# wenxichen/tensorflow_yolo2

Hardware: AMD Instinct MI355X
Metric: images/sec fwd+bwd Darknet-19 416x416 (higher is better)
Workload: dtype f16; 1 GPU; YOLO detector train step: darknet19_core + darknet19_detection(30) + get_loss + backward + Adam; image_size=416, batch_per_gpu=64, global_batch=64, S=13, B=2, parallelism=dp1, grad_allreduce=none

## Files before the change

### tensorflow_yolo2_amd/csrc/conv_halo.hip

```cpp
#include <stdio.h>
#include <stdlib.h>

#include <algorithm>

#include "common.h"
#include "conv_epilogue.h"
#include "kernels.h"

namespace y2 {

template <typename T, int WP, int WC, int TP, int TC, int BKB, int NSB, bool ADB>
struct HaloCfg {
    static constexpr int NW = WP * WC, NT = NW * 64;
    static constexpr int BP = WP * TP * 32, BC = WC * TC * 32;
    static constexpr int SZ = sizeof(T);
    static constexpr int LPR = BKB / 16, RPI = 64 / LPR, RPB = 256 / BKB;
    static constexpr int NI_C = BC / RPI;
    static constexpr int IPWB = (NI_C + NW - 1) / NW;
    static constexpr int IPW_MIN = NI_C / NW;
    static constexpr int BSTAGE = BC * BKB;
    static constexpr int KG = BKB / 32;
    static constexpr int NA = ADB ? 2 : 1;
};

// ... 403 lines not shown
    if (dtype == 3 && !no_pl2 && kb == 64) k128 = true;
    const int bkb = k128 ? 128 : 64;
    if (a.Cout > 64) {
        constexpr long kCUs = 256;
        const long wgs = (long)((a.M + 127) / 128) * ((a.Cout + 127) / 128);
        return conv_tile(2, 4, 2, 1, bkb, !dtype_split(dtype) && k128 && wgs <= kCUs ? 3 : 2);
    }
    return a.Cout > 32 ? conv_tile(4, 1, 2, 2, bkb, 2) : conv_tile(4, 1, 2, 1, bkb, 2);
}

#ifdef Y2_DEVBUILD
static int dev_rule(int W, int Cout) {
    static int n = -1;
    static int rules[32][3];
    if (n < 0) {
        n = 0;
        const char* e = getenv("Y2DEV_CONV");
        while (e && *e && n < 32) {
            int w, c, v, used = 0;
            if (sscanf(e, "%d:%d:%d%n", &w, &c, &v, &used) != 3) break;
            rules[n][0] = w; rules[n][1] = c; rules[n][2] = v; ++n;
            e += used;
            if (*e == ',') ++e;
        }
    }
    for (int i = 0; i < n; ++i)
        if (rules[i][0] == W && rules[i][1] == Cout) return rules[i][2];
    return -1;
}
#endif

static ConvPlan plan_route(int dtype, const ConvArgs& a) {
    ConvPlan p{CK_IGEMM, 0, 0, 0, 1};
    const int kb = a.C * dtype_kbytes(dtype);
    const bool split = dtype_split(dtype);
    const int rf = rf_config(a.taps, a.W, kb, a.Cout, a.M);
    const int rfn = rfn_config(a.taps, a.W, kb, a.Cout, a.M, a.is_dgrad, a.bw_psum != nullptr);
    if ((dtype == 1 || dtype == 2) && ((!a.bw_psum && rf) || rfn)) {
        p.kind = rf && !a.bw_psum ? CK_RF : CK_RFN;
        p.cfg = p.kind == CK_RF ? rf : rfn;
        const RfForm f = rf_form(p.cfg, a.bw_psum != nullptr);
        const int ntiles = (int)(((long)a.N * (a.H + 1) * (a.W + 1) + f.bp - 1) / f.bp);
        const int nblk = std::min((f.lds <= 80 * 1024 ? 512 : 256) / ((a.Cout + f.bc - 1) / f.bc), ntiles);
        p.rf_tiles = (ntiles + nblk - 1) / nblk;
        p.records = (ntiles + p.rf_tiles - 1) / p.rf_tiles;
        p.block_pixels = f.bp;
        p.lds = f.lds;
        return p;
    }
    if (a.taps == 9 && !(!split && (rf || rfn)) && (a.W <= 104 || a.Cout <= 32)) {
        p.kind = CK_HALOQ;
        p.cfg = haloq_tile(dtype, a, kb);
        p.filter_layout = ConvTile(p.cfg).aux ? 2 : 1;
        p.block_pixels = ConvTile(p.cfg).bp();
        if (p.cfg == HQ_256x64 && !split && a.M < 384 * 8) {
            const int depth = ks_clamp(ks_depth(((a.M + 255) / 256) * ((a.Cout + 63) / 64), 128, kb / 128), a);
            if (depth >= 2 && (size_t)image_rows(ConvTile(p.cfg), a, 0) * 128 <= (size_t)kLdsMax) {
                p.kind = CK_HALOQ_KS;
                p.ks_depth = depth;
                p.block_pixels = 128;
            }
        }
        return p;
    }
#ifdef Y2_DEVBUILD
    if (a.taps == 9 && dtype == 1 && dev_rule(a.W, a.Cout) >= 0) {
// ... 7 lines not shown
        p.kind = CK_HALO;
        p.cfg = halo_tile(dtype, a, kb);
        p.block_pixels = ConvTile(p.cfg).bp();
        return p;
    }
    p.cfg = igemm_tile(dtype, a, kb);
    p.block_pixels = ConvTile(p.cfg).bp();
    if (a.taps == 1 && dtype <= 2 && a.M < 384 * 8 && kb % 128 == 0 && a.Cout > 64) {
        const int depth = ks_clamp(ks_depth(((a.M + 127) / 128) * ((a.Cout + 127) / 128), 48, kb / 128), a);
        if (depth >= 2) {
            p.kind = CK_IGEMM_KS;
            p.cfg = conv_tile(2, 4, 2, 1, 128, 2);
            p.ks_depth = depth;
        }
    }
    return p;
}
ConvPlan plan_conv(int dtype, const ConvArgs& a) {
    ConvPlan p = plan_route(dtype, a);
    if (p.kind != CK_RF && p.kind != CK_RFN) p.records = (a.M + p.block_pixels - 1) / p.block_pixels;
    return p;
}

hipError_t launch_conv(int dtype, const ConvArgs& a0, hipStream_t s, int filter_layout) {
    static const int xcd_mode = getenv("Y2_XCD_CONV") ? atoi(getenv("Y2_XCD_CONV")) : 1;
    ConvArgs a = a0;
    a.xcd = xcd_mode;
    const ConvPlan p = plan_conv(dtype, a);
    if (filter_layout != p.filter_layout) return hipErrorInvalidValue;
    switch (p.kind) {
        case CK_RF: case CK_RFN: return launch_conv_rf(dtype, p, a, s);
        case CK_HALOQ: case CK_HALOQ_KS: return launch_conv_haloq(dtype, p, a, s);
        case CK_HALO: return launch_conv_halo(dtype, p, a, s);
        default: return launch_conv_igemm(dtype, p, a, s);
    }
}

#ifdef Y2_DEVBUILD
#define HV(id, WP, TPARGS...) \
    case id: if (bp) *bp = halo_bp<WP, TPARGS>(); return run ? halo_pick<T, WP, TPARGS>(a, s) : hipSuccess;
template <int WP, int WC, int TP, int TC, int BKB, int NSB, int ABL = 0>
static constexpr int halo_bp() { return WP * TP * 32; }
hipError_t launch_conv_halo_variant(int variant, const ConvArgs& a, hipStream_t s, int* bp, bool run) {
    typedef half_t T;
    switch (variant) {
        HV(86, 4, 2, 4, 1, 64, 2)
        HV(87, 4, 2, 3, 1, 64, 2)
        HV(88, 4, 2, 2, 1, 64, 2)
        HV(89, 4, 1, 4, 1, 128, 2)
        HV(90, 8, 1, 2, 1, 128, 2)
        HV(91, 8, 1, 4, 1, 128, 2)
        HV(92, 8, 1, 2, 1, 64, 2)
        HV(93, 8, 1, 4, 1, 64, 2)
        HV(94, 4, 2, 4, 2, 128, 2)
        HV(95, 8, 1, 2, 2, 128, 2)
        HV(96, 8, 1, 2, 2, 64, 2)
        HV(20, 2, 2, 2, 2, 128, 3)
        HV(21, 2, 2, 2, 2, 128, 2)
        HV(22, 2, 4, 2, 1, 128, 3)
        HV(23, 2, 4, 2, 1, 128, 2)
        HV(24, 4, 2, 2, 2, 128, 3)
        HV(25, 2, 4, 2, 2, 128, 3)
        HV(26, 2, 4, 2, 2, 128, 2)
        HV(27, 2, 2, 2, 2, 128, 4)
        HV(28, 2, 2, 2, 2, 64, 3)
        HV(29, 2, 2, 2, 2, 64, 2)
// ... 52 lines not shown
```

### tensorflow_yolo2_amd/csrc/kernels.h

```cpp
#pragma once
#include <hip/hip_runtime.h>
#include <stddef.h>
#include <stdint.h>
#include "../../include/yolo2_hip.h"

namespace y2 {

inline size_t dtype_size(int dtype) { return (dtype == 0 || dtype >= 3) ? 4 : 2; }
inline int dtype_kbytes(int dtype) { return dtype == 0 ? 4 : 2; }
inline bool dtype_split(int dtype) { return dtype >= 3; }
inline int dtype_plain(int dtype) { return dtype >= 3 ? 0 : dtype; }

struct ConvArgs {
    const void* x;
    const void* w;
    void* y;
    const float* bias;
    float* part_cnt;
    float* part_mean;
    float* part_m2;
    int N, H, W, C;
    int M;
    int Cout;
    int ldy;
    int taps;
    const void* bw_y = nullptr;
    const float* bw_scale = nullptr;
    const float* bw_shift = nullptr;
    float* bw_psum = nullptr;
    float bw_slope = 0.1f;
    unsigned* nonfinite = nullptr;
    int xcd = 0;
    int is_dgrad = 0;
    const float* aff_scale = nullptr;
    const float* aff_shift = nullptr;
    void* aff_out = nullptr;
    float aff_slope = 0.1f;
    uint32_t aff_magW = 0, aff_magH = 0;
    int aff_shW = 0, aff_shH = 0;
    int aff_pool = 0;
    float* ks_scratch = nullptr;
    size_t ks_floats = 0;
    int ks_splits = 0;
};
size_t conv_ks_scratch_floats(int taps, int M, int ldy, int row_bytes);
inline void conv_div_magic(uint32_t d, uint32_t* mag, int* sh) {
    int l = 0;
    while ((1u << l) < d) ++l;
    *sh = 31 + l;
    *mag = (uint32_t)((((uint64_t)1 << (31 + l)) + d - 1) / d);
}
inline void conv_set_affine(ConvArgs& a, const float* scale, const float* shift, void* out_bordered) {
    a.aff_scale = scale; a.aff_shift = shift; a.aff_out = out_bordered;
    conv_div_magic((uint32_t)a.W, &a.aff_magW, &a.aff_shW);
    conv_div_magic((uint32_t)a.H, &a.aff_magH, &a.aff_shH);
}

enum ConvKind {
    CK_RF,
    CK_RFN,
    CK_HALOQ,
    CK_HALOQ_KS,
    CK_HALO,
    CK_IGEMM,
    CK_IGEMM_KS,
};
struct ConvPlan {
    ConvKind kind;
    int cfg;
    int filter_layout;
    int block_pixels;
    int ks_depth;
    int records;
    int rf_tiles;
    int lds;
};
constexpr int rf_lds(int sz, int C, int nct, int wp, int tp, int pr) {
    return 4 * wp * tp * 32 * C * sz + wp * pr * (nct * 32 * sz + 16) + wp * (2 * nct * 32 + 2) * 8 + nct * 32 * 4;
}
constexpr int rfn_lds(int sz, int C, int wp, int wn, int tp, int nslot, bool bw) {
    const int bp = wp * tp * 32, bc = wn * 32, nw = wp * wn;
    return nslot * bp * C * sz + bp * (bc * sz + 16) + 2 * (nw * 2 * bc + nw) * 4 + bp * 4 + bc * 4 +
           (bw ? bp * bc * sz + 2 * bc * 4 : 0);
}
constexpr int conv_tile(int wp, int wc, int tp, int tc, int bkb, int aux) {
    return wp | wc << 4 | tp << 8 | tc << 12 | (bkb / 64) << 16 | aux << 20;
}
struct ConvTile {
    int wp, wc, tp, tc, bkb, aux;
    explicit ConvTile(int t)
        : wp(t & 15), wc((t >> 4) & 15), tp((t >> 8) & 15), tc((t >> 12) & 15), bkb(((t >> 16) & 15) * 64), aux(t >> 20) {}
    int bp() const { return wp * tp * 32; }
    int bc() const { return wc * tc * 32; }
};
ConvPlan plan_conv(int dtype, const ConvArgs& a);
hipError_t launch_conv(int dtype, const ConvArgs& a, hipStream_t s, int filter_layout);
hipError_t launch_conv_rf(int dtype, const ConvPlan& p, const ConvArgs& a, hipStream_t s);
hipError_t launch_conv_haloq(int dtype, const ConvPlan& p, const ConvArgs& a, hipStream_t s);
hipError_t launch_conv_halo(int dtype, const ConvPlan& p, const ConvArgs& a, hipStream_t s);
hipError_t launch_conv_igemm(int dtype, const ConvPlan& p, const ConvArgs& a, hipStream_t s);
int halo_image_rows(int H, int W, int BP, int RPI, int pool = 0);
int conv_block_couts(int Cout);
int mx8_block_couts();
int mx8_channels(int C);
struct Mx8Out {
    uint8_t* q = nullptr;
    uint8_t* sc = nullptr;
    int ldq = 0;
};
hipError_t launch_conv_mx8(int out_f32, const ConvArgs& a, const uint8_t* xsc, const uint8_t* wsc, const Mx8Out* qo,
                           hipStream_t s);
hipError_t launch_mx_unpack(const uint8_t* q, const uint8_t* sc, float* out, int N, int H, int W, int C, int Cs,
                            hipStream_t s);
hipError_t launch_mx_quantize(int in_f16, const void* x, size_t rows, int ldin, int ldq, uint8_t* q, uint8_t* sc,
                              hipStream_t s);
hipError_t launch_mx_pack_filter(const float* w, int taps, int Cin, int Cout, int Cout_pad, int C8, uint8_t* q,
                                 uint8_t* sc, hipStream_t s);

enum Conv1Fwd {
    C1F_PLAIN,
    C1F_POOLED,
};
enum Conv1Stats {
    C1S_NONE,
    C1S_CONV,
    C1S_GRAM,
};
enum Conv1Keep {
    C1K_NONE,
    C1K_Y,
    C1K_YSEL,
    C1K_IDX3,
};
// ... 412 lines not shown
```

### tensorflow_yolo2_amd/csrc/net.hip

```cpp
#include <math.h>
#include <stdarg.h>
#include <stdio.h>
#include <string.h>

#include <algorithm>
#include <string>
#include <vector>

#include "../../include/yolo2_hip.h"
#include "common.h"
#include "kernels.h"
#include "optim_math.h"

using namespace y2;

static thread_local std::string g_err;
namespace y2 {
int set_error(int code, const char* msg) {
    g_err = msg;
    return code;
}
}
static int fail(int code, const char* fmt, ...) {
    char buf[512];
// ... 7 lines not shown
#define HIPCHK(expr)                                                                                  \
    do {                                                                                              \
        hipError_t _e = (expr);                                                                       \
        if (_e != hipSuccess) return fail(Y2_ERR_HIP, "%s: %s (%s:%d)", #expr, hipGetErrorString(_e), \
                                          __FILE__, __LINE__);                                        \
    } while (0)

static inline size_t align_up(size_t v, size_t a) { return (v + a - 1) / a * a; }
static inline int round_up(int v, int a) { return (v + a - 1) / a * a; }

static inline size_t part_rows_bound(int N, int H, int W, int cout) {
    const size_t bp = 64;
    return ((size_t)N * (H + 1) * (W + 1) + bp - 1) / bp;
}

struct PadGeom {
    int N, H, W, C;
    size_t front_px() const { return (size_t)W + 3; }
    size_t body_px() const { return bbody_pixels(N, H, W); }
    size_t back_px() const { return (size_t)2 * W + 6 + 256; }
    size_t bytes(size_t sz) const { return align_up((front_px() + body_px() + back_px()) * C * sz + 64, 256); }
    size_t base_off(size_t sz) const { return front_px() * C * sz; }
};

struct Layer {
    int k, cin, cout, pool;
    int H, W, Ho, Wo, M;
    int cin_s;
    int ldy;
    int cout_pad;
    int cin_pad;
    bool first3;
    int wf_frag = 0, wd_frag = 0;
    float slope = 0.1f;
    size_t pW, pb, pg, pbeta;
    size_t smm, smv;
    size_t xin, y, stat, wf, wd, dyp, ysel, idx0;
    int cin8 = 0;
    size_t x8 = 0, x8s = 0, w8 = 0, w8s = 0;
};

enum FwdFold { FOLD_NONE, FOLD_AFFINE, FOLD_AFFINE_POOL };
enum FwdStats {
    FS_MOVING,
    FS_CONV,
    FS_SUB,
    FS_GRAM,
};
enum FwdApply {
    FA_NONE,
    FA_ACT,
    FA_FIN_ACT,
    FA_CONV1_POOL,
};
enum FwdOut { OUT_NEXT, OUT_EXT, OUT_F32, OUT_H32 };
enum BwdReduce {
    BR_KERNEL,
    BR_DGRAD,
    BR_CONV1_LIN,
    BR_CONV1_RECOMPUTE,
};
enum BwdApply { BA_FIN_APPLY, BA_FIN_THEN_APPLY, BA_FIN };
enum WgradRoute { WG_GENERIC, WG_CONV1, WG_CONV1_FUSED, WG_CONV1_LIN };
struct LayerPlan {
    int training = 0;
    bool mx8 = false;
    bool in8 = false;
    bool out8 = false;
    FwdFold fold = FOLD_NONE;
    FwdStats stats = FS_MOVING;
    int P = 0;
    FwdApply apply = FA_ACT;
    FwdOut out = OUT_NEXT;
    BwdReduce bred = BR_KERNEL;
    int bP = 0;
    BwdApply bapply = BA_FIN_THEN_APPLY;
    WgradRoute wgrad = WG_GENERIC;
    bool wgrad_side = false;
    bool dgrad = false;
    int dgrad_dtype = 0;
    bool dgrad_fuse = false;
    bool dgrad_guard = false;
    ConvPlan dgrad_plan{};
};
struct NetPlan {
    int train_core = 0, train_head = 0;
    std::vector<LayerPlan> L;
    Conv1Plan c1{};
};

struct y2_ctx {
    int N, H, W, dtype, tail, tail_k, core_layers;
    int bwd_dtype = 0;
    int fp8 = 0;
    int mx8_all = 0;
    std::vector<Layer> L;
    size_t nparams = 0, nstate = 0;
    int outN, outH, outW, outC;
    float grad_scale = 1.f;
    int bessel = 0;
    float bn_eps = 1e-3f, bn_momentum = 0.99f;
    int zero_bias_grad = 0;
// ... 53 lines not shown
    std::vector<ProfRec> prof_recs;
    size_t prof_used = 0;
    size_t sz() const { return dtype_size(dtype); }
    PadGeom in_geom(int l) const { return PadGeom{N, L[l].H, L[l].W, L[l].cin_s}; }
    PadGeom dy_geom(int l) const { return PadGeom{N, L[l].H, L[l].W, L[l].ldy}; }
    Conv1Plan conv1_plan(bool trains, bool training) const {
        const Layer& y = L[0];
        return plan_conv1(dtype, bwd_dtype, N, y.H, y.W, y.pool, y.cout, y.ldy, trains, L.size() > 1, training);
    }
};

enum { CAT_CONV_FWD = 0, CAT_CONV1_FWD, CAT_DGRAD, CAT_WGRAD, CAT_CONV1_WGRAD, CAT_BN_FWD, CAT_BN_BWD, CAT_MISC,
       CAT_COUNT };

struct ProfScope {
    y2_ctx* c; hipStream_t s; int idx = -1;
    ProfScope(y2_ctx* c_, hipStream_t s_, int cat) : c(c_), s(s_) {
        if (!c->prof) return;
        if (c->prof == 2 && cat != CAT_CONV_FWD && cat != CAT_DGRAD && cat != CAT_WGRAD) return;
        if (c->prof_used == c->prof_recs.size()) {
            y2_ctx::ProfRec r; r.cat = cat;
            if (hipEventCreate(&r.a) != hipSuccess || hipEventCreate(&r.b) != hipSuccess) return;
            c->prof_recs.push_back(r);
        }
        idx = (int)c->prof_used++;
        c->prof_recs[idx].cat = cat;
        c->prof_recs[idx].layer = c->prof_layer;
        (void)hipEventRecord(c->prof_recs[idx].a, s);
    }
    ~ProfScope() { if (idx >= 0) (void)hipEventRecord(c->prof_recs[idx].b, s); }
};
#define PROF(cat) ProfScope _prof_scope(c, s, cat)

static ConvArgs fwd_args(const y2_ctx* c, int l, bool stats, FwdFold fold) {
    const Layer& y = c->L[l];
    const size_t sz = c->sz();
    ConvArgs a{};
    a.x = (l == 0 && c->ext_xin) ? (char*)c->ext_xin : c->ws + y.xin + c->in_geom(l).base_off(sz);
    a.w = c->ws + y.wf; a.y = c->ws + y.y; a.bias = c->params + y.pb;
    if (stats) {
        a.part_cnt = (float*)(c->ws + c->o_part_cnt); a.part_mean = (float*)(c->ws + c->o_part_mean);
        a.part_m2 = (float*)(c->ws + c->o_part_m2);
    }
    a.N = c->N; a.H = y.H; a.W = y.W; a.C = y.cin_s; a.M = y.M; a.Cout = y.cout; a.ldy = y.ldy;
    a.taps = y.k * y.k;
    if (c->ks_floats) { a.ks_scratch = (float*)(c->ws + c->o_ks); a.ks_floats = c->ks_floats; }
    if (fold != FOLD_NONE) {
        const float* stat = (const float*)(c->ws + y.stat);
        conv_set_affine(a, stat, stat + y.ldy, c->ws + c->L[l + 1].xin + c->in_geom(l + 1).base_off(sz));
        a.aff_slope = y.slope;
        a.aff_pool = fold == FOLD_AFFINE_POOL ? 1 : 0;
    }
    return a;
}
static ConvArgs dgrad_args(const y2_ctx* c, int l, bool fuse, bool guard) {
    const Layer& y = c->L[l];
    ConvArgs a{};
    a.x = c->ws + y.dyp + c->dy_geom(l).base_off(c->sz()); a.w = c->ws + y.wd;
    a.N = c->N; a.H = y.H; a.W = y.W; a.C = y.ldy; a.M = y.M; a.Cout = y.cin; a.ldy = y.cin;
    a.taps = y.k * y.k;
    a.is_dgrad = 1;
    if (c->ks_floats) { a.ks_scratch = (float*)(c->ws + c->o_ks); a.ks_floats = c->ks_floats; }
    if (guard) a.nonfinite = (unsigned*)(c->ws + c->o_nfflag);
    if (fuse) {
        const Layer& z = c->L[l - 1];
        float* zs = (float*)(c->ws + z.stat);
        a.bw_y = c->ws + (z.pool ? z.ysel : z.y);
        a.bw_scale = zs; a.bw_shift = zs + z.ldy; a.bw_psum = (float*)(c->ws + c->o_psum);
        a.bw_slope = z.slope;
    }
    return a;
}
static int dgrad_dtype(const y2_ctx* c, int l) {
    return c->bwd_dtype == 4 && l > 0 && !c->L[l - 1].first3 ? 5 : c->bwd_dtype;
}

static bool mx8_speed_ok(int k, int cin, int cout, int pool, int H, int W) {
    return k == 3 && cin == 128 && cout == 256 && pool == 1 && H * W <= 28 * 28;
}
static bool mx8_shape(const y2_ctx* c, int l) {
    const Layer& y = c->L[l];
    if (!c->fp8 || y.first3 || y.pool == 2 || y.cin % 32 != 0) return false;
    if (c->mx8_all) return true;
    return mx8_speed_ok(y.k, y.cin, y.cout, y.pool, y.H, y.W);
}
static bool mx8_layer(const y2_ctx* c, int l, int training) {
    return !training && !c->bound_training && mx8_shape(c, l);
}

static NetPlan plan_net(const y2_ctx* c, int train_core, int train_head, int layer_lo, int layer_hi) {
    static const bool no_infer_fold = getenv("Y2_NO_INFER_FOLD") != nullptr;
    static const bool no_pool_fold = getenv("Y2_NO_POOL_FOLD") != nullptr;
    static const bool no_fin_fuse = getenv("Y2_NO_BN_FIN_FUSE") != nullptr;
    static const bool no_bnbwd_fuse = getenv("Y2_NO_BNBWD_FUSE") != nullptr;
    static const bool no_overlap = getenv("Y2_NO_WGRAD_OVERLAP") != nullptr;
    static const bool no_mx8 = getenv("Y2_NO_MX8") != nullptr;
    const int nl = (int)c->L.size();
    NetPlan n;
    n.train_core = train_core; n.train_head = train_head;
    n.L.resize(nl);
    for (int l = 0; l < nl; ++l) {
        const Layer& y = c->L[l];
        LayerPlan& p = n.L[l];
        p.training = l < c->core_layers ? train_core : train_head;
        p.out = l + 1 < nl ? OUT_NEXT : c->ext_out ? OUT_EXT : c->tail == Y2_TAIL_AVGPOOL ? OUT_H32 : OUT_F32;
        if (y.first3) {
            n.c1 = c->conv1_plan(c->bound_training, p.training);
            p.stats = !p.training ? FS_MOVING : n.c1.stats == C1S_GRAM ? FS_GRAM : FS_CONV;
            p.P = n.c1.fwd_blocks;
            p.apply = n.c1.fwd == C1F_POOLED ? FA_CONV1_POOL : FA_ACT;
        } else if (c->fp8 && !no_mx8 && mx8_layer(c, l, p.training)) {
            p.mx8 = true;
            p.stats = FS_MOVING;
            if (l + 1 < nl && y.pool == 0 && y.ldy == c->L[l + 1].cin_s && !no_infer_fold && y.M < 0x7FFFFFFF)
                p.fold = FOLD_AFFINE;
            p.apply = p.fold != FOLD_NONE ? FA_NONE : FA_ACT;
            if (l > 0 && n.L[l - 1].mx8 && n.L[l - 1].fold == FOLD_AFFINE) n.L[l - 1].out8 = p.in8 = true;
        } else {
            p.stats = !p.training ? FS_MOVING : y.pool == 2 ? FS_SUB : FS_CONV;
            const ConvPlan cp = plan_conv(c->dtype, fwd_args(c, l, p.stats == FS_CONV, FOLD_NONE));
            p.P = p.stats == FS_SUB ? bn_stats_sub_records(c->N, y.H, y.W) : cp.records;
            const bool fold = !p.training && l + 1 < nl && !c->bound_training && y.ldy == c->L[l + 1].cin_s &&
                              !no_infer_fold && !dtype_split(c->dtype) && cp.kind != CK_RF &&
                              !(cp.kind == CK_RFN && y.ldy % 8 != 0) && y.M < 0x7FFFFFFF;
            if (fold && y.pool == 0) p.fold = FOLD_AFFINE;
            if (fold && y.pool == 1 && !no_pool_fold && y.k == 3 && !(y.H & 1) && !(y.W & 1) && y.M >= 384 * 8 &&
                cp.kind == CK_HALOQ)
                p.fold = FOLD_AFFINE_POOL;
            if (p.fold != FOLD_NONE && plan_conv(c->dtype, fwd_args(c, l, false, p.fold)).filter_layout != y.wf_frag)
                p.fold = FOLD_NONE;
            p.apply = p.fold != FOLD_NONE ? FA_NONE : FA_ACT;
        }
        if (p.apply == FA_ACT && (p.stats == FS_CONV || p.stats == FS_SUB) && !no_fin_fuse &&
            (p.out == OUT_NEXT || p.out == OUT_EXT) && p.P >= 1 && p.P <= kBnFinPmax && y.ldy % kBnSlab == 0 &&
            y.cout == y.ldy)
            p.apply = FA_FIN_ACT;
    }
    bool forked = false;
    for (int l = layer_hi - 1; l >= layer_lo; --l) {
        const Layer& y = c->L[l];
        LayerPlan& p = n.L[l];
        const Conv1Bwd b1 = y.first3 ? n.c1.bwd : C1B_GENERIC;
        if (b1 == C1B_LINEAR) {
            p.bred = BR_CONV1_LIN;
            p.bP = n.c1.lin_records;
        } else if (b1 == C1B_RECOMPUTE) {
            p.bred = BR_CONV1_RECOMPUTE;
            p.bP = n.c1.pool_blocks;
        } else if (l + 1 < layer_hi && n.L[l + 1].dgrad_fuse) {
            p.bred = BR_DGRAD;
            p.bP = n.L[l + 1].dgrad_plan.records;
        } else {
            BnBwdArgs b{};
            b.N = c->N; b.H = y.H; b.W = y.W; b.C = y.cout; b.ldy = y.ldy; b.ldd = y.ldy; b.pool = y.pool;
            p.bred = BR_KERNEL;
            p.bP = bn_bwd_reduce_records(y.first3 ? dtype_plain(c->dtype) : c->dtype, b);
        }
        if (b1 == C1B_FUSED || b1 == C1B_LINEAR) p.bapply = BA_FIN;
        else if (!no_fin_fuse && p.bP >= 1 && p.bP <= kBnFinPmax && y.ldy % kBnSlab == 0 && y.cout == y.ldy)
            p.bapply = BA_FIN_APPLY;
        else p.bapply = BA_FIN_THEN_APPLY;
        if (y.first3) {
            p.wgrad = b1 == C1B_LINEAR ? WG_CONV1_LIN : b1 == C1B_FUSED ? WG_CONV1_FUSED : WG_CONV1;
            continue;
// ... 323 lines not shown
    return Y2_OK;
}
int y2_output_shape(const y2_ctx* c, int shape[4]) {
    shape[0] = c->outN; shape[1] = c->outH; shape[2] = c->outW; shape[3] = c->outC;
    return Y2_OK;
}
size_t y2_workspace_bytes(const y2_ctx* c, int training) { return training ? c->total_train : c->total_infer; }

int y2_bind(y2_ctx* c, float* params, float* grads, float* state, void* workspace, size_t workspace_bytes,
            int training, void* stream) {
    if (!params || !state || !workspace) return fail(Y2_ERR_ARG, "null buffer");
    if (training && !grads) return fail(Y2_ERR_ARG, "training needs a gradient buffer");
    if (training && c->fp8) return fail(Y2_ERR_ARG, "Y2_FP8 contexts are inference only: bind with training = 0");
    const size_t need = y2_workspace_bytes(c, training);
    if (workspace_bytes < need) return fail(Y2_ERR_ARG, "workspace too small: %zu < %zu", workspace_bytes, need);
    c->params = params; c->grads = grads; c->state = state;
    c->ws = (char*)workspace; c->ws_bytes = workspace_bytes; c->bound_training = training;
    c->weights_dirty = true; c->fwd_saved = false;
    ++c->bind_gen;
    HIPCHK(hipMemsetAsync(workspace, 0, need, (hipStream_t)stream));
    c->packtab.clear();
    int nb = 0, ntile = 0;
    for (size_t l = 0; l < c->L.size(); ++l) {
        Layer& y = c->L[l];
        if (y.first3) continue;
        PackLayer p{};
        p.W = params + y.pW;
        p.w_off = y.pW;
        p.wf = c->ws + y.wf;
        p.wd = training ? (void*)(c->ws + y.wd) : nullptr;
        p.taps = y.k * y.k; p.Cin = y.cin; p.Cout = y.cout; p.Cout_pad = y.cout_pad; p.Kc = y.cin_s;
        p.Cin_pad = y.cin_pad; p.Cdy = y.ldy;
        const int split = dtype_split(c->dtype) ? 1 : 0;
        p.wf_frag = y.wf_frag = plan_conv(c->dtype, fwd_args(c, (int)l, false, FOLD_NONE)).filter_layout;
        p.wd_frag = y.wd_frag = plan_conv(dgrad_dtype(c, (int)l), dgrad_args(c, (int)l, false, false)).filter_layout;
        pack_layer_plan(p, nb, split ? 2 : (int)c->sz());
        nb += p.wf_blocks + p.wd_blocks;
        p.opt_first = ntile;
        ntile += p.wf_blocks;
        c->packtab.push_back(p);
    }
    c->pack_blocks = nb;
    c->opt_tile_blocks = ntile;
    {
        std::vector<unsigned> rg;
        for (size_t l = 1; l <= c->L.size(); ++l) {
            const Layer& y = c->L[l % c->L.size()];
            rg.push_back((unsigned)y.pb);
            rg.push_back((unsigned)(3 * y.cout));
            rg.push_back(0u);
        }
        c->n_small_upper = (int)c->L.size() - 1;
        if (c->L[0].first3) {
            rg.push_back((unsigned)c->L[0].pW);
            rg.push_back((unsigned)(27 * c->L[0].cout));
            rg.push_back(1u);
        }
        c->n_smallranges = (int)(rg.size() / 3);
        HIPCHK(hipMemcpyAsync(c->ws + c->o_smallranges, rg.data(), rg.size() * sizeof(unsigned), hipMemcpyHostToDevice,
                              (hipStream_t)stream));
    }
    {
        std::vector<SgdSeg>& sg = c->sgdsegs;
        sg.clear();
        unsigned nblk = 0;
        for (const Layer& y : c->L) {
            const size_t nW = (size_t)y.k * y.k * y.cin * y.cout;
// ... 202 lines not shown
                if (images_u8) HIPCHK(launch_pack_input_u8(c->dtype, images_u8, xin, c->N, y.H, y.W, s));
                else HIPCHK(launch_pack_input(c->dtype, images, xin, c->N, y.H, y.W, s));
            }
            Conv1Args a{};
            a.x4 = xin; a.w = c->ws + y.wf; a.y = c->ws + y.y; a.bias = c->params + y.pb;
            a.part_cnt = part_cnt; a.part_mean = part_mean; a.part_m2 = part_m2;
            a.N = c->N; a.H = y.H; a.W = y.W; a.M = y.M;
            if (p.apply != FA_CONV1_POOL || p1.stats == C1S_CONV) { PROF(CAT_CONV1_FWD); HIPCHK(launch_conv1_fwd(p1, a, s)); }
        } else {
            if (l == 0 && !c->ext_xin) HIPCHK(launch_pack_act(c->dtype, images, xin, c->N, y.H, y.W, y.cin, y.cin_s, s));
            if (p.mx8) {
                const PadGeom g8{c->N, y.H, y.W, y.cin8}, gs{c->N, y.H, y.W, y.cin8 / 32};
                uint8_t* x8 = (uint8_t*)(c->ws + y.x8);
                uint8_t* x8s = (uint8_t*)(c->ws + y.x8s);
                if (!p.in8) {
                    PROF(CAT_MISC);
                    HIPCHK(launch_mx_quantize(1, xin - c->in_geom(l).base_off(sz), g8.front_px() + g8.body_px() + g8.back_px(),
                                              y.cin_s, y.cin8, x8, x8s, s));
                }
                ConvArgs a = fwd_args(c, l, false, p.fold);
                a.x = x8 + g8.base_off(1); a.C = y.cin8; a.w = c->ws + y.w8;
                a.ks_scratch = nullptr; a.ks_floats = 0;
                Mx8Out qo{};
                if (p.out8) {
                    const Layer& z = c->L[l + 1];
                    qo.q = (uint8_t*)(c->ws + z.x8) + PadGeom{c->N, z.H, z.W, z.cin8}.base_off(1);
                    qo.sc = (uint8_t*)(c->ws + z.x8s) + PadGeom{c->N, z.H, z.W, z.cin8 / 32}.base_off(1);
                    qo.ldq = z.cin8;
                }
                PROF(CAT_CONV_FWD);
                HIPCHK(launch_conv_mx8(0, a, x8s + gs.base_off(1), (const uint8_t*)(c->ws + y.w8s), p.out8 ? &qo : nullptr, s));
            } else {
                PROF(CAT_CONV_FWD);
                HIPCHK(launch_conv(c->dtype, fwd_args(c, l, p.stats == FS_CONV, p.fold), s, y.wf_frag));
            }
            if (p.stats == FS_SUB) {
                PROF(CAT_BN_FWD);
                HIPCHK(launch_bn_stats_sub(c->dtype, c->ws + y.y, c->N, y.H, y.W, y.ldy, part_cnt, part_mean, part_m2, s));
            }
        }
        if (p.apply == FA_NONE) continue;
        PROF(CAT_BN_FWD);
        BnFinalizeArgs f{};
        if (p.training) {
            f.part_cnt = part_cnt; f.part_mean = part_mean; f.part_m2 = part_m2;
            f.P = p.P; f.C = y.cout; f.ldp = y.first3 ? 32 : y.ldy;
            f.gamma = c->params + y.pg; f.beta = c->params + y.pbeta;
            f.moving_mean = c->state + y.smm; f.moving_var = c->state + y.smv;
            f.scale = scale; f.shift = shift; f.mean = mean; f.invstd = invstd;
            f.var = stat + 6 * y.ldy;
            f.scratch = (float*)(c->ws + c->o_part_scratch);
            f.eps = c->bn_eps; f.momentum = c->bn_momentum; f.update_moving = update_moving ? 1 : 0; f.bessel = c->bessel;
        }
        if (p.stats == FS_GRAM) {
            Conv1GramStatsArgs q{};
            q.x4 = xin; q.N = c->N; q.H = y.H; q.Wd = y.W;
            q.W = c->params + y.pW; q.bias = c->params + y.pb; q.gamma = f.gamma; q.beta = f.beta;
            q.moving_mean = f.moving_mean; q.moving_var = f.moving_var;
            q.scale = scale; q.shift = shift; q.mean = mean; q.invstd = invstd; q.var = f.var;
            q.eps = f.eps; q.momentum = f.momentum; q.update_moving = f.update_moving; q.bessel = f.bessel;
            q.gram = (float*)(c->ws + c->o_gram); q.mid = q.gram + 48 * 48;
            HIPCHK(launch_conv1_gram_stats(p1, q, s));
        } else if (p.stats != FS_MOVING && p.apply != FA_FIN_ACT) {
            HIPCHK(launch_bn_finalize(f, s));
        }
        if (p.apply == FA_CONV1_POOL) {
            Conv1PoolArgs q{};
            q.x4 = xin; q.w = c->ws + y.wf; q.y = c->ws + y.y; q.bias = c->params + y.pb;
            q.scale = scale; q.shift = shift;
            q.out = c->ws + c->L[l + 1].xin + c->in_geom(l + 1).base_off(sz);
            q.N = c->N; q.H = y.H; q.W = y.W;
            q.out_split = dtype_split(c->dtype) ? 1 : 0;
            if (p1.keep == C1K_IDX3) q.idx3 = (unsigned*)(c->ws + y.idx0);
            if (p1.keep == C1K_YSEL) { q.ysel = c->ws + y.ysel; q.idx = (unsigned short*)(c->ws + y.idx0); }
            HIPCHK(launch_conv1_pool(p1, q, s));
            continue;
        }
        BnActArgs b{};
        b.y = c->ws + y.y; b.scale = scale; b.shift = shift;
        b.N = c->N; b.H = y.H; b.W = y.W; b.C = y.cout; b.ldy = y.ldy; b.pool = y.pool;
        b.slope = y.slope;
        const void* join_t = c->ext_join_self ? (const void*)(c->ext_xin ? (char*)c->ext_xin : c->ws + c->L[0].xin + c->in_geom(0).base_off(sz))
                                              : c->ext_join;
        switch (p.out) {
            case OUT_NEXT: b.out = c->ws + c->L[l + 1].xin + c->in_geom(l + 1).base_off(sz); break;
            case OUT_EXT: b.out = c->ext_out; b.join_t = join_t; break;
            case OUT_F32: case OUT_H32:
                b.out = p.out == OUT_H32 ? (void*)(c->ws + c->o_h32) : (void*)out;
                b.out_f32 = 1;
                b.join = join;
                if (!join) b.join_t = join_t;
                break;
        }
        if (y.pool && c->bound_training && y.ysel) b.ysel = c->ws + y.ysel;
        if (p.apply == FA_FIN_ACT) HIPCHK(launch_bn_fin_act(c->dtype, b, f, s));
        else HIPCHK(launch_bn_act(c->dtype, b, s));
    }
    if (c->tail == Y2_TAIL_AVGPOOL) {
// ... 258 lines not shown
                                 y.cin_s, s));
    } else if (what == 1) {
        if (!c->fwd_saved) return fail(Y2_ERR_STATE, "run y2_forward first");
        if (c->fwd.L[l].fold != FOLD_NONE)
            return fail(Y2_ERR_STATE, "layer %d: inference batch norm was folded into the convolution, its conv output "
                                      "is not stored (Y2_NO_INFER_FOLD=1 keeps the two-pass form)", l);
        const Conv1Plan& p = c->fwd.c1;
        if (y.first3 && !p.y_stored && p.bwd != C1B_LINEAR)
            return fail(Y2_ERR_STATE, "inference binding: the pooled first layer does not store its conv output");
        if (y.first3 && !p.y_stored) {
            Conv1Plan q = p;
            q.fwd = C1F_PLAIN;
            Conv1Args a{};
            a.x4 = c->ws + y.xin + c->in_geom(l).base_off(sz); a.w = c->ws + y.wf; a.y = c->ws + y.y;
            a.bias = c->params + y.pb;
            a.part_cnt = (float*)(c->ws + c->o_part_cnt); a.part_mean = (float*)(c->ws + c->o_part_mean);
            a.part_m2 = (float*)(c->ws + c->o_part_m2);
            a.N = c->N; a.H = y.H; a.W = y.W; a.M = y.M;
            HIPCHK(launch_conv1_fwd(q, a, s));
        }
        HIPCHK(launch_cast_to_f32(c->dtype, c->ws + y.y, dst, (size_t)y.M, y.cout, y.ldy, s));
    } else if (what == 2) {
        if (!c->bound_training) return fail(Y2_ERR_STATE, "no gradients in inference binding");
        if (y.first3 && (!c->fwd_saved || !c->fwd.c1.dy_stored))
            return fail(Y2_ERR_STATE, "the first layer's dy is fused into its weight gradient and never stored");
        HIPCHK(launch_unpack_act(y.first3 ? dtype_plain(c->dtype) : c->dtype, c->ws + y.dyp + c->dy_geom(l).base_off(sz), dst, c->N, y.H, y.W, y.cout,
                                 y.ldy, s));
    } else if (what == 3) {
        if (!c->fwd_saved) return fail(Y2_ERR_STATE, "run y2_forward first");
        const float* stat = (const float*)(c->ws + y.stat);
        const float* src[4] = {stat + 2 * y.ldy, stat + 3 * y.ldy, stat, stat + y.ldy};
        for (int k = 0; k < 4; ++k)
            HIPCHK(hipMemcpyAsync(dst + (size_t)k * y.cout, src[k], (size_t)y.cout * sizeof(float), hipMemcpyDeviceToDevice, s));
    } else {
        return fail(Y2_ERR_ARG, "unknown selector");
    }
    return Y2_OK;
}

size_t y2_yolo_loss_workspace_bytes(int batch, int S) { return (size_t)loss_blocks(batch, S) * 4 * sizeof(float) + 256; }

int y2_yolo_loss(const float* net, const float* labels, int num_class, int batch, float image_size, int S, int B,
                 float lambda_coord, float lambda_noobj, float* loss, float* ious, float* object_mask, float* dnet,
                 void* workspace, void* stream) {
    if (!net || !labels || !loss || !ious || !object_mask || !workspace) return fail(Y2_ERR_ARG, "null tensor");
    if (B < 1 || B > 8 || num_class < 1 || S < 1 || batch < 1) return fail(Y2_ERR_ARG, "bad loss geometry");
    LossArgs a{};
    a.net = net; a.labels = labels; a.loss = loss; a.ious = ious; a.mask = object_mask; a.dnet = dnet;
    a.partial = (float*)workspace;
    a.N = batch; a.S = S; a.B = B; a.C = num_class; a.image_size = image_size;
    a.lambda_coord = lambda_coord; a.lambda_noobj = lambda_noobj;
    HIPCHK(launch_yolo_loss(a, (hipStream_t)stream));
    return Y2_OK;
}
int y2_get_iou(const float* b1, const float* b2, float* iou, int n, void* stream) {
    if (!b1 || !b2 || !iou || n < 0) return fail(Y2_ERR_ARG, "bad arguments");
    if (n == 0) return Y2_OK;
    HIPCHK(launch_get_iou(b1, b2, iou, n, (hipStream_t)stream));
    return Y2_OK;
}
int y2_decode_detections(const float* predict, int S, int B, int num_class, int im_w, int im_h, float thresh,
                         int* det, float* conf, void* stream) {
    if (!predict || !det || !conf) return fail(Y2_ERR_ARG, "null tensor");
    HIPCHK(launch_decode(predict, S, B, num_class, im_w, im_h, thresh, det, conf, (hipStream_t)stream));
    return Y2_OK;
}
// ... 343 lines not shown
```

### tensorflow_yolo2_amd/engine.py

```python
import ctypes as C
import os

import numpy as np
import torch

from . import _lib
from ._lib import check

CORE_SPEC = [
    (3, 3, 32, 1),
    (3, 32, 64, 1),
    (3, 64, 128, 0), (3, 128, 64, 0), (3, 64, 128, 1),
    (3, 128, 256, 0), (1, 256, 128, 0), (3, 128, 256, 1),
    (3, 256, 512, 0), (1, 512, 256, 0), (3, 256, 512, 0), (1, 512, 256, 0), (3, 256, 512, 1),
    (3, 512, 1024, 0), (1, 1024, 512, 0), (3, 512, 1024, 0), (1, 1024, 512, 0), (3, 512, 1024, 0),
]


def det_head_spec(output_filter):
    return [(3, 1024, 1024, 0)] * 3 + [(1, 1024, output_filter, 0)]


CLS_HEAD_SPEC = [(1, 1024, 1000, 0)]

# ... 253 lines not shown

    def wait_mark(self, k, stream):
        check(self.lib.y2_wait_mark(self.h, int(k), C.c_void_p(stream.cuda_stream)))

    def profile_enable(self, on=1):
        check(self.lib.y2_profile_enable(self.h, int(on)))

    def profile_busy(self, categories=("conv_fwd", "dgrad", "wgrad")):
        mask = sum(1 << self.PROFILE_CATEGORIES.index(k) for k in categories)
        ms, n = C.c_double(), C.c_int()
        check(self.lib.y2_profile_busy(self.h, mask, C.byref(ms), C.byref(n)))
        return ms.value, n.value

    def profile_layers(self):
        buf = (C.c_double * (self.num_layers * len(self.PROFILE_CATEGORIES)))()
        check(self.lib.y2_profile_layers(self.h, buf))
        return np.array(buf).reshape(self.num_layers, len(self.PROFILE_CATEGORIES))

    def profile_collect(self):
        n = len(self.PROFILE_CATEGORIES)
        ms = (C.c_double * n)()
        cnt = (C.c_int * n)()
        check(self.lib.y2_profile_collect(self.h, ms, cnt, n))
        return {k: (ms[i], cnt[i]) for i, k in enumerate(self.PROFILE_CATEGORIES)}

    def layer_statistics(self, layer):
        co = self.spec[layer][2]
        t = torch.empty((4, co), dtype=torch.float32, device=self.device)
        check(self.lib.y2_debug_read(self.h, layer, 3, _ptr(t), _stream()))
        a = t.double().cpu().numpy()
        eps = self.bn_eps
        return {"mean": a[0], "invstd": a[1], "scale": a[2], "shift": a[3], "var": 1.0 / (a[1] * a[1]) - eps}

    def debug_read(self, layer, what):
        k, ci, co, _ = self.spec[layer]
        info = (C.c_int * 8)()
        check(self.lib.y2_layer_info(self.h, layer, info))
        c = ci if what == 0 else co
        t = torch.empty((self.batch, info[4], info[5], c), dtype=torch.float32, device=self.device)
        check(self.lib.y2_debug_read(self.h, layer, what, _ptr(t), _stream()))
        return t


class Bordered:

    def __init__(self, n, h, w, c, dtype, device):
        lib = _lib.load()
        dt = _lib.DTYPES[dtype] if isinstance(dtype, str) else int(dtype)
        if dt not in (_lib.Y2_F32, _lib.Y2_F16, _lib.Y2_BF16):
            raise ValueError("Bordered: linked tensors exist in f32 / f16 / bf16 (not the split-operand modes f16x2 / f16x2f)")
        off = C.c_size_t(0)
        nbytes = lib.y2_bordered_bytes(n, h, w, c, dt, C.byref(off))
        self.buf = torch.zeros(nbytes, dtype=torch.uint8, device=device)
        self.cell0 = self.buf.data_ptr() + off.value
        self.shape = (n, h, w, c)
        self._off, self._tdtype = off.value, {_lib.Y2_F32: torch.float32, _lib.Y2_F16: torch.float16, _lib.Y2_BF16: torch.bfloat16}[dt]

    def _interior(self):
        n, h, w, c = self.shape
        esz = torch.empty(0, dtype=self._tdtype).element_size()
        rows = n * (h + 1)
        body = self.buf[self._off:self._off + rows * (w + 1) * c * esz].view(self._tdtype).view(n, h + 1, w + 1, c)
        return body[:, 1:, 1:, :]

    def write(self, x):
        self._interior().copy_(x.to(self._tdtype))
# ... 861 lines not shown
```

Measured before the change: 7803 images/s.

## Fuse previous layer's BN+leaky apply into following 1x1 conv prologue

Adds a pointwise conv kernel that reads the previous layer's raw conv output, applies batch-norm scale/shift and leaky ReLU in its prologue, and writes the activated bordered input while also staging it in LDS for the MFMA GEMM. The separate BN-apply pass for the producer layer is skipped when the pair qualifies. This removes one full read and write of the activation tensor for selected 3x3→1x1 pairs (256→128 and 512→256) in training. In exchange it uses a new hand-written GEMM kernel that may be less efficient than the existing conv paths, and it adds planning complexity.

Result: no change. 7847 images/s (median of 6 runs) (+0.6%).

```diff
diff --git a/tensorflow_yolo2_amd/csrc/conv_halo.hip b/tensorflow_yolo2_amd/csrc/conv_halo.hip
--- a/tensorflow_yolo2_amd/csrc/conv_halo.hip
+++ b/tensorflow_yolo2_amd/csrc/conv_halo.hip
@@ -459,6 +459,12 @@
 
 static ConvPlan plan_route(int dtype, const ConvArgs& a) {
     ConvPlan p{CK_IGEMM, 0, 0, 0, 1};
+    if (a.pw_y && conv_pw_shape_ok(dtype, a)) {
+        p.kind = CK_PW;
+        p.filter_layout = 2;
+        p.block_pixels = kPwBP;
+        return p;
+    }
     const int kb = a.C * dtype_kbytes(dtype);
     const bool split = dtype_split(dtype);
     const int rf = rf_config(a.taps, a.W, kb, a.Cout, a.M);
@@ -532,6 +538,7 @@
         case CK_RF: case CK_RFN: return launch_conv_rf(dtype, p, a, s);
         case CK_HALOQ: case CK_HALOQ_KS: return launch_conv_haloq(dtype, p, a, s);
         case CK_HALO: return launch_conv_halo(dtype, p, a, s);
+        case CK_PW: return launch_conv_pw(dtype, p, a, s);
         default: return launch_conv_igemm(dtype, p, a, s);
     }
 }
diff --git a/tensorflow_yolo2_amd/csrc/conv_pw.hip b/tensorflow_yolo2_amd/csrc/conv_pw.hip
--- /dev/null
+++ b/tensorflow_yolo2_amd/csrc/conv_pw.hip
@@ -0,0 +1,189 @@
+#include <stdlib.h>
+#include "common.h"
+#include "conv_epilogue.h"
+#include "kernels.h"
+
+namespace y2 {
+
+namespace {
+constexpr int kPwU = 4;
+constexpr int kPwLdsMax = 160 * 1024;
+
+struct PwGeom {
+    uint32_t magW, magH;
+    int shW, shH;
+    int wtiles;
+};
+
+template <typename T, int WC, int TC, int KC>
+struct PwCfg {
+    static constexpr int NT = WC * 64, K = KC * 128, CPR = K / 8, RSTEP = NT / CPR, NR = kPwBP / RSTEP;
+    static constexpr int IMAGE = kPwBP * K * 2;
+    typedef EpiCfg<T, 1, WC, 2, TC> Epi;
+    static constexpr int LDS = IMAGE > Epi::LDS ? IMAGE : Epi::LDS;
+    static_assert(NT % CPR == 0 && kPwBP % RSTEP == 0, "a thread keeps one channel chunk over its pixel rows");
+    static_assert(sizeof(T) == 2, "16-bit types");
+};
+
+template <typename T, int WC, int TC, int KC>
+__global__ __launch_bounds__(WC * 64, (16 * KC / WC <= 8 && TC == 1 ? 4 : 2)) void bn_act_pw_kernel(ConvArgs a, PwGeom g) {
+    typedef PwCfg<T, WC, TC, KC> Cfg;
+    typedef typename Elem<T>::frag frag_t;
+    constexpr int K = Cfg::K, CPR = Cfg::CPR, RSTEP = Cfg::RSTEP, NR = Cfg::NR, EPC = 8, ROWB = K * 2;
+    constexpr int NA = 2 * TC, NB = 4, U = kPwU, NG = K / 32 / U;
+    extern __shared__ __attribute__((aligned(16))) char smem[];
+
+    const int tid = threadIdx.x;
+    const int lane = tid & 63;
+    const int w = __builtin_amdgcn_readfirstlane(tid >> 6);
+    const int pt = blockIdx.x, m0 = pt * kPwBP;
+
+    const int r16 = lane & 15, g4 = lane >> 4;
+    const char* wrow[NA];
+#pragma unroll
+    for (int i = 0; i < NA; ++i) {
+        int tile = w * NA + i;
+        if (tile > g.wtiles - 1) tile = g.wtiles - 1;
+        wrow[i] = (const char*)a.w + ((size_t)tile * (K / 32) * 64 + lane) * 16;
+    }
+    auto load_group = [&](int grp, frag_t (&f)[U][NA]) {
+#pragma unroll
+        for (int u = 0; u < U; ++u)
+#pragma unroll
+            for (int i = 0; i < NA; ++i) f[u][i] = *(const frag_t*)(wrow[i] + (grp * U + u) * 1024);
+    };
+    frag_t fa0[U][NA], fa1[U][NA];
+    constexpr bool EARLY2 = KC == 8;
+    load_group(0, fa0);
+    if (EARLY2 && NG > 1) load_group(1, fa1);
+
+    {
+        const int ch = tid % CPR, row0 = tid / CPR;
+        const int c0 = ch * EPC;
+        float sc[EPC], sh[EPC];
+#pragma unroll
+        for (int e = 0; e < EPC; ++e) {
+            sc[e] = a.pw_scale[c0 + e];
+            sh[e] = a.pw_shift[c0 + e];
+        }
+        Chunk<T> v[NR];
+#pragma unroll
+        for (int j = 0; j < NR; ++j) {
+            int m = m0 + row0 + j * RSTEP;
+            if (m > a.M - 1) m = a.M - 1;
+            v[j] = ld_chunk<T>((const char*)a.pw_y + ((size_t)m * K + c0) * sizeof(T));
+        }
+#pragma unroll
+        for (int j = 0; j < NR; ++j) {
+            const int p = row0 + j * RSTEP;
+            const uint32_t m = (uint32_t)(m0 + p);
+            Chunk<T> o;
+            if ((int)m < a.M) {
+                float r[EPC];
+#pragma unroll
+                for (int e = 0; e < EPC; ++e) r[e] = leaky_s(Elem<T>::to_f32(v[j].v[e]) * sc[e] + sh[e], a.pw_slope);
+#pragma unroll
+                for (int e = 0; e < EPC; ++e) o.v[e] = Elem<T>::from_f32(r[e]);
+                const uint32_t rr = (uint32_t)(((uint64_t)m * g.magW) >> g.shW);
+                const uint32_t n = (uint32_t)(((uint64_t)rr * g.magH) >> g.shH);
+                const size_t bp = (size_t)m + rr + (size_t)(n + 1) * (uint32_t)(a.W + 1) + 1;
+                st_chunk<T>((char*)a.pw_x + (bp * K + c0) * sizeof(T), o);
+            } else {
+#pragma unroll
+                for (int e = 0; e < EPC; ++e) o.v[e] = (T)0.0f;
+            }
+            st_chunk<T>(smem + p * ROWB + ((ch ^ (p & 15)) * 16), o);
+        }
+    }
+    asm volatile("s_waitcnt lgkmcnt(0)" ::: "memory");
+    __builtin_amdgcn_s_barrier();
+    asm volatile("" ::: "memory");
+
+    const char* prow = smem + r16 * ROWB;
+    f32x4 acc[NA][NB];
+#pragma unroll
+    for (int i = 0; i < NA; ++i)
+#pragma unroll
+        for (int j = 0; j < NB; ++j) acc[i][j] = f32x4{0.f, 0.f, 0.f, 0.f};
+
+    auto mma_group = [&](int grp, frag_t (&f)[U][NA]) {
+#pragma unroll
+        for (int u = 0; u < U; ++u) {
+            const int ks = grp * U + u;
+            frag_t fb[NB];
+#pragma unroll
+            for (int j = 0; j < NB; ++j) fb[j] = *(const frag_t*)(prow + j * 16 * ROWB + (((ks * 4 + g4) ^ r16) * 16));
+#pragma unroll
+            for (int i = 0; i < NA; ++i)
+#pragma unroll
+                for (int j = 0; j < NB; ++j) mma16(acc[i][j], f[u][i], fb[j]);
+        }
+    };
+    if (!EARLY2 && NG > 1) load_group(1, fa1);
+    for (int grp = 0; grp < NG; grp += 2) {
+        mma_group(grp, fa0);
+        if (grp + 2 < NG) load_group(grp + 2, fa0);
+        if (grp + 1 < NG) {
+            mma_group(grp + 1, fa1);
+            if (grp + 3 < NG) load_group(grp + 3, fa1);
+        }
+    }
+    __syncthreads();
+
+    conv_epilogue16<T, 1, WC, 2, TC>(a, acc, smem, w, lane, m0, 0, pt, 0);
+}
+
+template <typename T, int WC, int TC, int KC>
+hipError_t pw_launch(const ConvArgs& a, const PwGeom& g, hipStream_t s) {
+    typedef PwCfg<T, WC, TC, KC> Cfg;
+    static_assert(Cfg::LDS <= kPwLdsMax, "LDS budget");
+    void (*kern)(ConvArgs, PwGeom) = bn_act_pw_kernel<T, WC, TC, KC>;
+    static bool attr_set = false;
+    if (!attr_set) {
+        hipError_t e = hipFuncSetAttribute((const void*)kern, hipFuncAttributeMaxDynamicSharedMemorySize, Cfg::LDS);
+        if (e != hipSuccess) return e;
+        attr_set = true;
+    }
+    hipLaunchKernelGGL(kern, dim3((a.M + kPwBP - 1) / kPwBP), dim3(Cfg::NT), Cfg::LDS, s, a, g);
+    return hipGetLastError();
+}
+
+template <typename T>
+hipError_t pw_run(const ConvArgs& a, const PwGeom& g, hipStream_t s) {
+    const int bc = conv_pw_block_couts(a.Cout);
+#define PW(BC, WC, TC)                                              \
+    if (bc == BC) switch (a.C) {                                    \
+        case 128: return pw_launch<T, WC, TC, 1>(a, g, s);          \
+        case 256: return pw_launch<T, WC, TC, 2>(a, g, s);          \
+        case 512: return pw_launch<T, WC, TC, 4>(a, g, s);          \
+        case 1024: return pw_launch<T, WC, TC, 8>(a, g, s);         \
+    }
+    PW(128, 4, 1)
+    PW(256, 8, 1)
+    PW(512, 8, 2)
+#undef PW
+    return hipErrorInvalidValue;
+}
+}
+
+int conv_pw_block_couts(int Cout) { return Cout <= 128 ? 128 : Cout <= 256 ? 256 : Cout <= 512 ? 512 : 0; }
+
+bool conv_pw_shape_ok(int dtype, const ConvArgs& a) {
+    if (dtype != 1 && dtype != 2) return false;
+    if (a.taps != 1 || a.is_dgrad || a.bw_psum || a.aff_out || a.nonfinite) return false;
+    if (a.C != 128 && a.C != 256 && a.C != 512 && a.C != 1024) return false;
+    if (!conv_pw_block_couts(a.Cout) || a.ldy % 8 != 0 || a.M >= 0x7FFFFFFF - kPwBP) return false;
+    return true;
+}
+
+hipError_t launch_conv_pw(int dtype, const ConvPlan& p, const ConvArgs& a, hipStream_t s) {
+    if (p.kind != CK_PW || !a.pw_y || !a.pw_x || !a.pw_scale || !a.pw_shift || !conv_pw_shape_ok(dtype, a))
+        return hipErrorInvalidValue;
+    PwGeom g{};
+    conv_div_magic((uint32_t)a.W, &g.magW, &g.shW);
+    conv_div_magic((uint32_t)a.H, &g.magH, &g.shH);
+    g.wtiles = (a.Cout + conv_block_couts(a.Cout) - 1) / conv_block_couts(a.Cout) * conv_block_couts(a.Cout) / 16;
+    return dtype == 1 ? pw_run<half_t>(a, g, s) : pw_run<bf16_t>(a, g, s);
+}
+
+}
diff --git a/tensorflow_yolo2_amd/csrc/kernels.h b/tensorflow_yolo2_amd/csrc/kernels.h
--- a/tensorflow_yolo2_amd/csrc/kernels.h
+++ b/tensorflow_yolo2_amd/csrc/kernels.h
@@ -42,6 +42,11 @@
     float* ks_scratch = nullptr;
     size_t ks_floats = 0;
     int ks_splits = 0;
+    const void* pw_y = nullptr;
+    const float* pw_scale = nullptr;
+    const float* pw_shift = nullptr;
+    void* pw_x = nullptr;
+    float pw_slope = 0.1f;
 };
 size_t conv_ks_scratch_floats(int taps, int M, int ldy, int row_bytes);
 inline void conv_div_magic(uint32_t d, uint32_t* mag, int* sh) {
@@ -64,6 +69,7 @@
     CK_HALO,
     CK_IGEMM,
     CK_IGEMM_KS,
+    CK_PW,
 };
 struct ConvPlan {
     ConvKind kind;
@@ -99,6 +105,10 @@
 hipError_t launch_conv_haloq(int dtype, const ConvPlan& p, const ConvArgs& a, hipStream_t s);
 hipError_t launch_conv_halo(int dtype, const ConvPlan& p, const ConvArgs& a, hipStream_t s);
 hipError_t launch_conv_igemm(int dtype, const ConvPlan& p, const ConvArgs& a, hipStream_t s);
+hipError_t launch_conv_pw(int dtype, const ConvPlan& p, const ConvArgs& a, hipStream_t s);
+constexpr int kPwBP = 64;
+int conv_pw_block_couts(int Cout);
+bool conv_pw_shape_ok(int dtype, const ConvArgs& a);
 int halo_image_rows(int H, int W, int BP, int RPI, int pool = 0);
 int conv_block_couts(int Cout);
 int mx8_block_couts();
diff --git a/tensorflow_yolo2_amd/csrc/net.hip b/tensorflow_yolo2_amd/csrc/net.hip
--- a/tensorflow_yolo2_amd/csrc/net.hip
+++ b/tensorflow_yolo2_amd/csrc/net.hip
@@ -63,6 +63,7 @@
     int cin_pad;
     bool first3;
     int wf_frag = 0, wd_frag = 0;
+    bool pw = false;
     float slope = 0.1f;
     size_t pW, pb, pg, pbeta;
     size_t smm, smv;
@@ -83,6 +84,7 @@
     FA_ACT,
     FA_FIN_ACT,
     FA_CONV1_POOL,
+    FA_NEXT_PW,
 };
 enum FwdOut { OUT_NEXT, OUT_EXT, OUT_F32, OUT_H32 };
 enum BwdReduce {
@@ -99,6 +101,7 @@
     bool in8 = false;
     bool out8 = false;
     FwdFold fold = FOLD_NONE;
+    bool pw = false;
     FwdStats stats = FS_MOVING;
     int P = 0;
     FwdApply apply = FA_ACT;
@@ -218,7 +221,7 @@
 };
 #define PROF(cat) ProfScope _prof_scope(c, s, cat)
 
-static ConvArgs fwd_args(const y2_ctx* c, int l, bool stats, FwdFold fold) {
+static ConvArgs fwd_args(const y2_ctx* c, int l, bool stats, FwdFold fold, bool pw = false) {
     const Layer& y = c->L[l];
     const size_t sz = c->sz();
     ConvArgs a{};
@@ -236,6 +239,12 @@
         conv_set_affine(a, stat, stat + y.ldy, c->ws + c->L[l + 1].xin + c->in_geom(l + 1).base_off(sz));
         a.aff_slope = y.slope;
         a.aff_pool = fold == FOLD_AFFINE_POOL ? 1 : 0;
+    }
+    if (pw) {
+        const Layer& z = c->L[l - 1];
+        const float* zs = (const float*)(c->ws + z.stat);
+        a.pw_y = c->ws + z.y; a.pw_scale = zs; a.pw_shift = zs + z.ldy; a.pw_slope = z.slope;
+        a.pw_x = c->ws + y.xin + c->in_geom(l).base_off(sz);
     }
     return a;
 }
@@ -272,6 +281,25 @@
 }
 static bool mx8_layer(const y2_ctx* c, int l, int training) {
     return !training && !c->bound_training && mx8_shape(c, l);
+}
+
+static bool pw_speed_ok(int cin, int cout, int W);
+static bool pw_pair(const y2_ctx* c, int l) {
+    static const bool no_pw = getenv("Y2_NO_PW_FUSE") != nullptr;
+    static const int pw_min_m = getenv("Y2_PW_MIN_M") ? atoi(getenv("Y2_PW_MIN_M")) : 384 * 8;
+    static const bool pw_all = getenv("Y2_PW_ALL") != nullptr;
+    if (no_pw) return false;
+    if (l < 1 || (c->dtype != 1 && c->dtype != 2) || c->fp8 || !c->bound_training) return false;
+    const Layer &y = c->L[l], &z = c->L[l - 1];
+    if (y.k != 1 || y.cout < 64 || z.first3 || z.pool != 0 || z.ldy != y.cin_s || z.cout != z.ldy) return false;
+    if ((l - 1 < c->core_layers) != (l < c->core_layers)) return false;
+    if (y.M < pw_min_m || !(pw_all || pw_speed_ok(y.cin, y.cout, y.W))) return false;
+    const ConvPlan f = plan_conv(c->dtype, fwd_args(c, l, true, FOLD_NONE, true));
+    return f.kind == CK_PW && (size_t)f.records <= c->part_rows;
+}
+static bool pw_speed_ok(int cin, int cout, int W) {
+    (void)W;
+    return (cin == 256 && cout == 128) || (cin == 512 && cout == 256);
 }
 
 static NetPlan plan_net(const y2_ctx* c, int train_core, int train_head, int layer_lo, int layer_hi) {
@@ -316,6 +344,16 @@
             if (p.fold != FOLD_NONE && plan_conv(c->dtype, fwd_args(c, l, false, p.fold)).filter_layout != y.wf_frag)
                 p.fold = FOLD_NONE;
             p.apply = p.fold != FOLD_NONE ? FA_NONE : FA_ACT;
+            if (p.fold == FOLD_NONE && y.pw) {
+                LayerPlan& q = n.L[l - 1];
+                const ConvPlan f = plan_conv(c->dtype, fwd_args(c, l, p.stats == FS_CONV, FOLD_NONE, true));
+                if ((q.apply == FA_ACT || q.apply == FA_FIN_ACT) && q.out == OUT_NEXT && !q.mx8 && f.kind == CK_PW &&
+                    f.filter_layout == y.wf_frag) {
+                    p.pw = true;
+                    if (p.stats == FS_CONV) p.P = f.records;
+                    q.apply = FA_NEXT_PW;
+                }
+            }
         }
         if (p.apply == FA_ACT && (p.stats == FS_CONV || p.stats == FS_SUB) && !no_fin_fuse &&
             (p.out == OUT_NEXT || p.out == OUT_EXT) && p.P >= 1 && p.P <= kBnFinPmax && y.ldy % kBnSlab == 0 &&
@@ -705,7 +743,8 @@
         p.taps = y.k * y.k; p.Cin = y.cin; p.Cout = y.cout; p.Cout_pad = y.cout_pad; p.Kc = y.cin_s;
         p.Cin_pad = y.cin_pad; p.Cdy = y.ldy;
         const int split = dtype_split(c->dtype) ? 1 : 0;
-        p.wf_frag = y.wf_frag = plan_conv(c->dtype, fwd_args(c, (int)l, false, FOLD_NONE)).filter_layout;
+        y.pw = pw_pair(c, (int)l);
+        p.wf_frag = y.wf_frag = plan_conv(c->dtype, fwd_args(c, (int)l, false, FOLD_NONE, y.pw)).filter_layout;
         p.wd_frag = y.wd_frag = plan_conv(dgrad_dtype(c, (int)l), dgrad_args(c, (int)l, false, false)).filter_layout;
         pack_layer_plan(p, nb, split ? 2 : (int)c->sz());
         nb += p.wf_blocks + p.wd_blocks;
@@ -974,7 +1013,7 @@
                 HIPCHK(launch_conv_mx8(0, a, x8s + gs.base_off(1), (const uint8_t*)(c->ws + y.w8s), p.out8 ? &qo : nullptr, s));
             } else {
                 PROF(CAT_CONV_FWD);
-                HIPCHK(launch_conv(c->dtype, fwd_args(c, l, p.stats == FS_CONV, p.fold), s, y.wf_frag));
+                HIPCHK(launch_conv(c->dtype, fwd_args(c, l, p.stats == FS_CONV, p.fold, p.pw), s, y.wf_frag));
             }
             if (p.stats == FS_SUB) {
                 PROF(CAT_BN_FWD);
@@ -1006,6 +1045,7 @@
         } else if (p.stats != FS_MOVING && p.apply != FA_FIN_ACT) {
             HIPCHK(launch_bn_finalize(f, s));
         }
+        if (p.apply == FA_NEXT_PW) continue;
         if (p.apply == FA_CONV1_POOL) {
             Conv1PoolArgs q{};
             q.x4 = xin; q.w = c->ws + y.wf; q.y = c->ws + y.y; q.bias = c->params + y.pb;
@@ -1330,6 +1370,9 @@
         const float* src[4] = {stat + 2 * y.ldy, stat + 3 * y.ldy, stat, stat + y.ldy};
         for (int k = 0; k < 4; ++k)
             HIPCHK(hipMemcpyAsync(dst + (size_t)k * y.cout, src[k], (size_t)y.cout * sizeof(float), hipMemcpyDeviceToDevice, s));
+    } else if (what == 4) {
+        if (!c->fwd_saved) return fail(Y2_ERR_STATE, "run y2_forward first");
+        HIPCHK(launch_fill(dst, 1, c->fwd.L[l].pw ? 1.0f : 0.0f, s));
     } else {
         return fail(Y2_ERR_ARG, "unknown selector");
     }
diff --git a/tensorflow_yolo2_amd/engine.py b/tensorflow_yolo2_amd/engine.py
--- a/tensorflow_yolo2_amd/engine.py
+++ b/tensorflow_yolo2_amd/engine.py
@@ -309,6 +309,11 @@
         eps = self.bn_eps
         return {"mean": a[0], "invstd": a[1], "scale": a[2], "shift": a[3], "var": 1.0 / (a[1] * a[1]) - eps}
 
+    def forward_fused(self, layer):
+        t = torch.empty((1,), dtype=torch.float32, device=self.device)
+        check(self.lib.y2_debug_read(self.h, layer, 4, _ptr(t), _stream()))
+        return bool(t.item() == 1.0)
+
     def debug_read(self, layer, what):
         k, ci, co, _ = self.spec[layer]
         info = (C.c_int * 8)()
```
